# mengcaopku/DCNet

Hardware: AMD Instinct MI355X
Metric: clips/sec (T=8, 416x416, bs8) fwd+bwd (higher is better)
Workload: dtype f32; 1 GPU; T=8 416x416 bs8/GPU L=20 fp32, 64 img/GPU/step as pairs, fwd+5 losses+bwd+RMSprop; arith=f16x2-split MFMA, fp32 accumulate, parallelism=dp1, ranks_seen=1, reducer=none, step=hipGraph replay (fwd+losses+bwd+RMSprop), sampler=mt

## Files before the change

dcnet_amd/csrc/coattn.hip:

```cpp
#include "igemm.h"
#include "prof.h"
#include "coattn.h"

int tn_gemm_batched(const float* A, int lda, long long a_bs, const float* B, int ldb, long long b_bs,
                    float* C, int ldc, long long c_bs, const float* row_scale,
                    int M, int m_ld, int N, int K, int batch, int accumulate, hipStream_t stream,
                    const unsigned* amax_a = nullptr, const unsigned* amax_b = nullptr);

namespace {

constexpr int EXP_ROWS = 32;

typedef _Float16 f16x4c_t __attribute__((ext_vector_type(4)));
constexpr float E_SPLIT_SCALE = 8192.f;
template <bool SPLIT>
__global__ __launch_bounds__(256) void exp_sums_kernel(float* __restrict__ E, int hw, int ldE, float t,
                                                       float* __restrict__ rsum, float* __restrict__ colpart) {
  __shared__ float red[4][EXP_ROWS];
  const int b = blockIdx.y, rb = blockIdx.x;
  const int i0 = rb * EXP_ROWS;
  float* e = E + ((size_t)b * hw + i0) * ldE;
  float racc[EXP_ROWS];
#pragma unroll
  for (int r = 0; r < EXP_ROWS; ++r) racc[r] = 0.f;
// ... 16 lines not shown
          const f16x4c_t l = {(_Float16)(ts[0] - (float)h[0]), (_Float16)(ts[1] - (float)h[1]), (_Float16)(ts[2] - (float)h[2]),
                              (_Float16)(ts[3] - (float)h[3])};
          unsigned char* run = reinterpret_cast<unsigned char*>(e + (size_t)r * ldE + (j & ~7)) + (j & 4) * 2;
          *reinterpret_cast<f16x4c_t*>(run) = h;
          *reinterpret_cast<f16x4c_t*>(run + 16) = l;
        } else {
          *reinterpret_cast<f32x4*>(e + (size_t)r * ldE + j) = o;
        }
        cs += o; racc[r] += (o[0] + o[1]) + (o[2] + o[3]);
      }
    }
    *reinterpret_cast<f32x4*>(colpart + ((size_t)rb * gridDim.y + b) * ldE + j) = cs;
  }
  const int lane = threadIdx.x & 63, wave = threadIdx.x >> 6;
#pragma unroll
  for (int r = 0; r < EXP_ROWS; ++r) {
    const float s = wave_sum(racc[r]);
    if (lane == 0) red[wave][r] = s;
  }
  __syncthreads();
  if (threadIdx.x < EXP_ROWS && i0 + threadIdx.x < hw)
    rsum[(size_t)b * hw + i0 + threadIdx.x] = 1.f / (red[0][threadIdx.x] + red[1][threadIdx.x] + red[2][threadIdx.x] + red[3][threadIdx.x]);
}

__global__ __launch_bounds__(256) void colsum_inv_kernel(const float* __restrict__ colpart, int nrb, int b, int hw, int ldE,
                                                         float* __restrict__ cinv) {
  const int j = blockIdx.x * 256 + threadIdx.x, bb = blockIdx.y;
  if (j >= hw) return;
  float s = 0.f;
  for (int rb = 0; rb < nrb; ++rb) s += colpart[((size_t)rb * b + bb) * ldE + j];
  cinv[(size_t)bb * hw + j] = 1.f / s;
}

enum { AM_ONE = 0, AM_DO1, AM_DO2, AM_DO1S, AM_DO2S, AM_DA, AM_DP1, AM_DP2, AM_SLOTS };
__global__ __launch_bounds__(256) void amax_init_kernel(unsigned* __restrict__ w) {
  for (int i = threadIdx.x; i < AM_SLOTS * DCN_AMAX_WORDS; i += 256) w[i] = i < DCN_AMAX_WORDS ? 0x3F800000u : 0u;
}

__global__ __launch_bounds__(256) void rowdot_scale_kernel(const float* __restrict__ d, int ldd, int64_t bsd,
                                                           const float* __restrict__ o, int ldo, int64_t bso, int hw,
                                                           const float* __restrict__ inv, int64_t rows, int c,
                                                           float* __restrict__ delta, float* __restrict__ ds,
                                                           unsigned* __restrict__ amax_d, unsigned* __restrict__ amax_ds) {
  __shared__ float red[4];
  const int lane = threadIdx.x & 63;
  const int64_t row = (int64_t)blockIdx.x * 4 + (threadIdx.x >> 6);
  float vmax = 0.f, s = 0.f;
  if (row < rows) {
    const int64_t bb = row / hw, i = row - bb * hw;
    s = inv[row];
    float acc = 0.f;
    for (int k = lane * 4; k < c; k += 256) {
      const f32x4 dv = *reinterpret_cast<const f32x4*>(d + bb * bsd + i * ldd + k);
      const f32x4 ov = *reinterpret_cast<const f32x4*>(o + bb * bso + i * ldo + k);
      acc += dv[0] * ov[0] + dv[1] * ov[1] + dv[2] * ov[2] + dv[3] * ov[3];
      *reinterpret_cast<f32x4*>(ds + row * c + k) = dv * s;
      vmax = fmaxf(fmaxf(vmax, fmaxf(fabsf(dv[0]), fabsf(dv[1]))), fmaxf(fabsf(dv[2]), fabsf(dv[3])));
    }
    acc = wave_sum(acc);
    if (lane == 0) delta[row] = acc;
  }
  const float vs = wave_max(vmax * s);
  amax_update_block(amax_d, vmax, red);
  __syncthreads();
  amax_update_block(amax_ds, vs, red);
}

template <bool ESPLIT, bool OSPLIT = false>
__global__ __launch_bounds__(256) void dA_kernel(const float* __restrict__ E, float* __restrict__ dP1, const float* __restrict__ dP2,
                                                 const float* __restrict__ rinv, const float* __restrict__ cinv,
                                                 const float* __restrict__ d1, const float* __restrict__ d2,
                                                 int hw, int ldE, float t, int64_t total4, unsigned* __restrict__ amax_da) {
  __shared__ float red[4];
  float vmax = 0.f;
  const int l4 = ldE >> 2;
  float s_out = 1.f;
  if constexpr (OSPLIT) {
    const int be = (int)((amax_read(amax_da) >> 23) & 0xFF);
    int ex = (be == 0 || be == 255) ? 0 : 14 - (be - 126);
    ex = ex > 100 ? 100 : (ex < -100 ? -100 : ex);
    s_out = __uint_as_float((unsigned)(ex + 127) << 23);
  }
  for (int64_t idx = (int64_t)blockIdx.x * 256 + threadIdx.x; idx < total4; idx += (int64_t)gridDim.x * 256) {
    const int64_t row = idx / l4;
    const int j = (int)(idx - row * l4) * 4;
    const int64_t bb = row / hw;
    f32x4 e;
    if constexpr (ESPLIT) {
      const unsigned char* run = reinterpret_cast<const unsigned char*>(E + row * ldE + (j & ~7)) + (j & 4) * 2;
      const f16x4c_t h = *reinterpret_cast<const f16x4c_t*>(run), l = *reinterpret_cast<const f16x4c_t*>(run + 16);
#pragma unroll
      for (int k = 0; k < 4; ++k) e[k] = ((float)h[k] + (float)l[k]) * (1.f / E_SPLIT_SCALE);
    } else {
      e = *reinterpret_cast<const f32x4*>(E + row * ldE + j);
    }
    const f32x4 p1 = *reinterpret_cast<const f32x4*>(dP1 + row * ldE + j);
    const f32x4 p2 = *reinterpret_cast<const f32x4*>(dP2 + row * ldE + j);
    const float ri = rinv[row], di = d1[row];
    f32x4 o;
#pragma unroll
    for (int k = 0; k < 4; ++k) {
      float v = 0.f;
      if (j + k < hw) v = t * e[k] * ((p1[k] - di) * ri + (p2[k] - d2[bb * hw + j + k]) * cinv[bb * hw + j + k]);
      o[k] = v;
    }
    if constexpr (OSPLIT) {
      const f32x4 ts = o * s_out;
      const f16x4c_t h = {(_Float16)ts[0], (_Float16)ts[1], (_Float16)ts[2], (_Float16)ts[3]};
      const f16x4c_t l = {(_Float16)(ts[0] - (float)h[0]), (_Float16)(ts[1] - (float)h[1]), (_Float16)(ts[2] - (float)h[2]),
                          (_Float16)(ts[3] - (float)h[3])};
      unsigned char* run = reinterpret_cast<unsigned char*>(dP1 + row * ldE + (j & ~7)) + (j & 4) * 2;
      *reinterpret_cast<f16x4c_t*>(run) = h;
      *reinterpret_cast<f16x4c_t*>(run + 16) = l;
    } else {
      *reinterpret_cast<f32x4*>(dP1 + row * ldE + j) = o;
      vmax = fmaxf(fmaxf(vmax, fmaxf(fabsf(o[0]), fabsf(o[1]))), fmaxf(fabsf(o[2]), fabsf(o[3])));
    }
  }
  if constexpr (!OSPLIT) amax_update_block(amax_da, vmax, red);
}

__global__ __launch_bounds__(64) void da_bound_kernel(const unsigned* __restrict__ a1, const unsigned* __restrict__ a2, float t,
                                                      unsigned* __restrict__ out) {
  const float b = 2.f * t * (__uint_as_float(amax_read(a1)) + __uint_as_float(amax_read(a2)));
  out[threadIdx.x & (DCN_AMAX_WORDS - 1)] = __float_as_uint(b);
}

inline int ld_pad(int hw) { return (hw + 31) / 32 * 32; }

void gemm_params(IgemmParams& p, const float* A, int lda, long long a_bs, const float* B, int ldb, long long b_bs,
                 float* C, int ldc, long long c_bs, int M, int N, int K, int batch) {
  p = IgemmParams{};
  p.osy = p.osx = p.isy = p.isx = 1; p.dense_out = 1;
  p.in = A; p.ldi = lda; p.in_bs = a_bs; p.wt = B; p.ldw = ldb; p.wt_bs = b_bs; p.out = C; p.ldo = ldc; p.out_bs = c_bs;
  p.ldr = ldc;
  p.N = 1; p.Hi = 1; p.Wi = M; p.Ho = 1; p.Wo = M; p.Hs = 1; p.Ws = M; p.M = M;
// ... 29 lines not shown
  return (int64_t)cdiv(hw, EXP_ROWS) * b * ld_pad(hw) + AM_SLOTS * DCN_AMAX_WORDS;
}
extern "C" int64_t dcn_coattn_e_size(int b, int hw) { return (int64_t)b * hw * ld_pad(hw); }
extern "C" int64_t dcn_coattn_saved_size(int b, int hw, int c) {
  return dcn_coattn_e_size(b, hw) + (on_gemm3(b, hw, c) ? (int64_t)2 * b * hw * c : 0);
}

extern "C" int dcn_coattn_fwd(const float* f1, const float* f2, int ldf, int64_t bsf, float* f1_attn, float* f2_attn, int ldo,
                              int64_t bso, float* E, float* rinv, float* cinv, float* ws,
                              int b, int hw, int c, float temperature, void* stream_) {
  hipStream_t stream = (hipStream_t)stream_;
  DCN_CHECK_ARG(f1 && f2 && f1_attn && E && rinv && cinv && ws, "coattn_fwd: null pointer");
  DCN_CHECK_ARG(b > 0 && hw > 0 && c > 0 && c % 32 == 0, "coattn_fwd: bad shape (c=%d must be a multiple of 32)", c);
  if (ldf <= 0) ldf = c;
  if (ldo <= 0) ldo = c;
  DCN_CHECK_ARG(ldf % 4 == 0 && ldo % 4 == 0, "coattn_fwd: ldf/ldo must be multiples of 4");
  if (bsf <= 0) bsf = (int64_t)hw * ldf;
  if (bso <= 0) bso = (int64_t)hw * ldo;
  DCN_CHECK_ARG(bsf % 4 == 0 && bso % 4 == 0, "coattn_fwd: batch strides must be multiples of 4");
  const int ldE = ld_pad(hw);
  unsigned* am = reinterpret_cast<unsigned*>(ws + (int64_t)cdiv(hw, EXP_ROWS) * b * ldE);
  hipLaunchKernelGGL(amax_init_kernel, dim3(1), dim3(256), 0, stream, am);
  DCN_CHECK_LAUNCH("coattn amax_init");
  const unsigned* one = am + AM_ONE * DCN_AMAX_WORDS;
  const int nrb = cdiv(hw, EXP_ROWS);
  const long long bsE = (long long)hw * ldE;
  if (on_gemm3(b, hw, c)) {
    float* f1s = E + dcn_coattn_e_size(b, hw);
    float* f2s = f1s + (int64_t)b * hw * c;
    const long long bss = (long long)hw * c;
    int rc = gemm3_presplit(f1, ldf, bsf, f1s, c, bss, b, hw, c, one, stream);
    if (rc) return rc;
    if ((rc = gemm3_presplit(f2, ldf, bsf, f2s, c, bss, b, hw, c, one, stream))) return rc;
    if ((rc = gemm3_launch(f1s, c, bss, 0, f2s, c, bss, 0, E, ldE, bsE, nullptr, 0, hw, hw, c, b, 0, one, one, stream))) return rc;
    const int pid = prof_begin(12, (double)b * hw * ldE * 8.0, stream);
    hipLaunchKernelGGL(exp_sums_kernel<true>, dim3(nrb, b), dim3(256), 0, stream, E, hw, ldE, temperature, rinv, ws);
    prof_end(pid, stream);
    DCN_CHECK_LAUNCH("exp_sums");
    hipLaunchKernelGGL(colsum_inv_kernel, dim3(cdiv(hw, 256), b), dim3(256), 0, stream, ws, nrb, b, hw, ldE, cinv);
    DCN_CHECK_LAUNCH("colsum_inv");
    if ((rc = gemm3_launch(E, ldE, bsE, 0, f2s, c, bss, 1, f1_attn, ldo, bso, rinv, hw, hw, c, hw, b, 0, one, one, stream))) return rc;
    if (f2_attn) rc = gemm3_launch(E, ldE, bsE, 1, f1s, c, bss, 1, f2_attn, ldo, bso, cinv, hw, hw, c, hw, b, 0, one, one, stream);
    return rc;
  }
  IgemmParams p;
  gemm_params(p, f1, ldf, bsf, f2, ldf, bsf, E, ldE, (long long)hw * ldE, hw, hw, c, b);
  p.amax_a = one; p.amax_b = one;
  int rc = igemm_launch(p, stream);
  if (rc) return rc;
  const int pid = prof_begin(12, (double)b * hw * ldE * 8.0, stream);
  hipLaunchKernelGGL(exp_sums_kernel<false>, dim3(nrb, b), dim3(256), 0, stream, E, hw, ldE, temperature, rinv, ws);
  prof_end(pid, stream);
  DCN_CHECK_LAUNCH("exp_sums");
  hipLaunchKernelGGL(colsum_inv_kernel, dim3(cdiv(hw, 256), b), dim3(256), 0, stream, ws, nrb, b, hw, ldE, cinv);
  DCN_CHECK_LAUNCH("colsum_inv");
  gemm_params(p, E, ldE, (long long)hw * ldE, f2, ldf, bsf, f1_attn, ldo, bso, hw, c, ldE, b);
  p.bmode = 1; p.kvalid = hw; p.row_scale = rinv; p.amax_a = one; p.amax_b = one;
  rc = igemm_launch(p, stream);
  if (rc) return rc;
  if (f2_attn)
    rc = tn_gemm_batched(E, ldE, (long long)hw * ldE, f1, ldf, bsf, f2_attn, ldo, bso,
                         cinv, hw, ldE, c, hw, b, 0, stream, one, one);
  return rc;
}

extern "C" int64_t dcn_coattn_bwd_ws(int b, int hw, int c) {
  return (int64_t)2 * b * hw * ld_pad(hw) + (int64_t)2 * b * hw * c + (int64_t)2 * b * hw + AM_SLOTS * DCN_AMAX_WORDS +
         (on_gemm3(b, hw, c) ? (int64_t)2 * b * hw * c + 4 : 0);
}

extern "C" int dcn_coattn_bwd(const float* f1, const float* f2, int ldf, int64_t bsf,
                              const float* d_f1_attn, const float* d_f2_attn, int lddo, int64_t bsdo,
                              const float* f1_attn, const float* f2_attn, int ldo, int64_t bso,
                              const float* E, const float* rinv, const float* cinv,
                              float* d_f1, float* d_f2, int lddf, int64_t bsdf, int accumulate, float* ws,
                              int b, int hw, int c, float temperature, void* stream_) {
  hipStream_t stream = (hipStream_t)stream_;
  DCN_CHECK_ARG(f1 && f2 && d_f1_attn && d_f2_attn && f1_attn && f2_attn && E && rinv && cinv && d_f1 && d_f2 && ws,
                "coattn_bwd: null pointer");
  DCN_CHECK_ARG(b > 0 && hw > 0 && c > 0 && c % 32 == 0, "coattn_bwd: bad shape");
  if (ldf <= 0) ldf = c;
  if (ldo <= 0) ldo = c;
  if (lddo <= 0) lddo = c;
  if (lddf <= 0) lddf = c;
  if (bsf <= 0) bsf = (int64_t)hw * ldf;
  if (bso <= 0) bso = (int64_t)hw * ldo;
  if (bsdo <= 0) bsdo = (int64_t)hw * lddo;
  if (bsdf <= 0) bsdf = (int64_t)hw * lddf;
  const int ldE = ld_pad(hw);
  const long long rows = (long long)b * hw;
  float* dP1 = ws;
  float* dP2 = dP1 + rows * ldE;
  float* dO1s = dP2 + rows * ldE;
  float* dO2s = dO1s + rows * c;
  float* del1 = dO2s + rows * c;
  float* del2 = del1 + rows;
  unsigned* am = reinterpret_cast<unsigned*>(del2 + rows);
  hipLaunchKernelGGL(amax_init_kernel, dim3(1), dim3(256), 0, stream, am);
  DCN_CHECK_LAUNCH("coattn amax_init");
  auto slot = [&](int i) { return am + i * DCN_AMAX_WORDS; };
  hipLaunchKernelGGL(rowdot_scale_kernel, dim3(cdiv(rows, 4)), dim3(256), 0, stream, d_f1_attn, lddo, bsdo, f1_attn, ldo, bso, hw, rinv, rows, c, del1, dO1s,
                     slot(AM_DO1), slot(AM_DO1S));
  DCN_CHECK_LAUNCH("rowdot_scale");
  hipLaunchKernelGGL(rowdot_scale_kernel, dim3(cdiv(rows, 4)), dim3(256), 0, stream, d_f2_attn, lddo, bsdo, f2_attn, ldo, bso, hw, cinv, rows, c, del2, dO2s,
                     slot(AM_DO2), slot(AM_DO2S));
  DCN_CHECK_LAUNCH("rowdot_scale");
  const int64_t total4 = rows * (ldE / 4);
  int64_t g = (total4 + 255) / 256; if (g > 8192) g = 8192;
  if (g > 1024) g = 1024;
  const long long bsE = (long long)hw * ldE;
  if (on_gemm3(b, hw, c)) {
    float* dO1p = reinterpret_cast<float*>(((uintptr_t)(am + AM_SLOTS * DCN_AMAX_WORDS) + 15) & ~(uintptr_t)15);
    float* dO2p = dO1p + rows * c;
    const float* f1s = E + dcn_coattn_e_size(b, hw);
    const float* f2s = f1s + rows * c;
    const long long bss = (long long)hw * c;
    int rc;
    if ((rc = gemm3_presplit(d_f1_attn, lddo, bsdo, dO1p, c, bss, b, hw, c, slot(AM_DO1), stream))) return rc;
    if ((rc = gemm3_presplit(d_f2_attn, lddo, bsdo, dO2p, c, bss, b, hw, c, slot(AM_DO2), stream))) return rc;
    if ((rc = gemm3_presplit(dO1s, c, bss, dO1s, c, bss, b, hw, c, slot(AM_DO1S), stream))) return rc;
    if ((rc = gemm3_presplit(dO2s, c, bss, dO2s, c, bss, b, hw, c, slot(AM_DO2S), stream))) return rc;
    if ((rc = gemm3_launch(dO1p, c, bss, 0, f2s, c, bss, 0, dP1, ldE, bsE, nullptr, 0, hw, hw, c, b, 0, slot(AM_DO1), slot(AM_ONE), stream, slot(AM_DP1)))) return rc;
    if ((rc = gemm3_launch(f1s, c, bss, 0, dO2p, c, bss, 0, dP2, ldE, bsE, nullptr, 0, hw, hw, c, b, 0, slot(AM_ONE), slot(AM_DO2), stream, slot(AM_DP2)))) return rc;
    hipLaunchKernelGGL(da_bound_kernel, dim3(1), dim3(64), 0, stream, slot(AM_DP1), slot(AM_DP2), temperature, slot(AM_DA));
    DCN_CHECK_LAUNCH("dA bound");
    const int pid_da = prof_begin(31, (double)total4 * 16.0 * 4.0, stream);
    hipLaunchKernelGGL((dA_kernel<true, true>), dim3((int)g), dim3(256), 0, stream, E, dP1, dP2, rinv, cinv, del1, del2, hw, ldE, temperature, total4, slot(AM_DA));
    prof_end(pid_da, stream);
    DCN_CHECK_LAUNCH("dA");
    if ((rc = gemm3_launch(dP1, ldE, bsE, 0, f2s, c, bss, 1, d_f1, lddf, bsdf, nullptr, 0, hw, c, hw, b, accumulate, slot(AM_DA), slot(AM_ONE), stream))) return rc;
    if ((rc = gemm3_launch(E, ldE, bsE, 0, dO2s, c, bss, 1, d_f1, lddf, bsdf, nullptr, 0, hw, c, hw, b, 1, slot(AM_ONE), slot(AM_DO2S), stream))) return rc;
    if ((rc = gemm3_launch(dP1, ldE, bsE, 1, f1s, c, bss, 1, d_f2, lddf, bsdf, nullptr, 0, hw, c, hw, b, accumulate, slot(AM_DA), slot(AM_ONE), stream))) return rc;
    return gemm3_launch(E, ldE, bsE, 1, dO1s, c, bss, 1, d_f2, lddf, bsdf, nullptr, 0, hw, c, hw, b, 1, slot(AM_ONE), slot(AM_DO1S), stream);
  }
  IgemmParams p;
  int rc;
  gemm_params(p, d_f1_attn, lddo, bsdo, f2, ldf, bsf, dP1, ldE, (long long)hw * ldE, hw, hw, c, b);
  p.amax_a = slot(AM_DO1); p.amax_b = slot(AM_ONE);
  if ((rc = igemm_launch(p, stream))) return rc;
  gemm_params(p, f1, ldf, bsf, d_f2_attn, lddo, bsdo, dP2, ldE, (long long)hw * ldE, hw, hw, c, b);
  p.amax_a = slot(AM_ONE); p.amax_b = slot(AM_DO2);
  if ((rc = igemm_launch(p, stream))) return rc;
  const int pid_da = prof_begin(31, (double)total4 * 16.0 * 4.0, stream);
  hipLaunchKernelGGL(dA_kernel<false>, dim3((int)g), dim3(256), 0, stream, E, dP1, dP2, rinv, cinv, del1, del2, hw, ldE, temperature, total4, slot(AM_DA));
  prof_end(pid_da, stream);
  DCN_CHECK_LAUNCH("dA");
  gemm_params(p, dP1, ldE, (long long)hw * ldE, f2, ldf, bsf, d_f1, lddf, bsdf, hw, c, ldE, b);
  p.bmode = 1; p.kvalid = hw; p.accumulate = accumulate; p.amax_a = slot(AM_DA); p.amax_b = slot(AM_ONE);
  if ((rc = igemm_launch(p, stream))) return rc;
  gemm_params(p, E, ldE, (long long)hw * ldE, dO2s, c, (long long)hw * c, d_f1, lddf, bsdf, hw, c, ldE, b);
  p.bmode = 1; p.kvalid = hw; p.accumulate = 1; p.amax_a = slot(AM_ONE); p.amax_b = slot(AM_DO2S);
  if ((rc = igemm_launch(p, stream))) return rc;
  rc = tn_gemm_batched(dP1, ldE, (long long)hw * ldE, f1, ldf, bsf, d_f2, lddf, bsdf,
                       nullptr, hw, ldE, c, hw, b, accumulate, stream, slot(AM_DA), slot(AM_ONE));
  if (rc) return rc;
  return tn_gemm_batched(E, ldE, (long long)hw * ldE, dO1s, c, (long long)hw * c, d_f2, lddf, bsdf,
                         nullptr, hw, ldE, c, hw, b, 1, stream, slot(AM_ONE), slot(AM_DO1S));
}
```

dcnet_amd/csrc/gemm3.hip:

```cpp
#include "igemm.h"
#include "prof.h"

namespace {

typedef _Float16 f16x8_t __attribute__((ext_vector_type(8)));
typedef short s16x4 __attribute__((ext_vector_type(4)));
typedef short s16x8 __attribute__((ext_vector_type(8)));
typedef __attribute__((address_space(3))) void lds_void;

#ifndef G3_ABL
#define G3_ABL 0
#endif
constexpr unsigned G3_OOB = 0x80000000u;
constexpr int G3_BM = 256, G3_BN = 256, G3_STAGES = 4;
constexpr int G3_TILE = 256 * 64;
constexpr int G3_STAGE = 2 * G3_TILE;
constexpr int G3_LDS = G3_STAGES * G3_STAGE;

__device__ __forceinline__ float g3_pow2_scale(unsigned amax_bits) {
  const int be = (int)((amax_bits >> 23) & 0xFF);
  if (be == 0 || be == 255) return 1.f;
  int e = 14 - (be - 126);
  e = e > 100 ? 100 : (e < -100 ? -100 : e);
  return __uint_as_float((unsigned)(e + 127) << 23);
}

struct G3Params {
  const float* A; const float* B; float* C;
  long long a_bs, b_bs, c_bs;
  int lda, ldb, ldc;
  int M, N, K;
  int a_rows, b_rows;
  int a_cols, b_cols;
  int tiles_m, tiles_n;
  const float* row_scale; long long rs_bs;
  int accumulate;
  const unsigned* amax_a; const unsigned* amax_b;
  unsigned* amax_out;
  int var;
  int abl;
};

__device__ __forceinline__ int g3_tswz(int krow) { return (krow & 1) | ((krow & 2) << 1); }

template <bool AT, bool BT, bool H1 = false>
__global__ __launch_bounds__(512, 1) void gemm3_kernel(const G3Params p) {
  extern __shared__ __attribute__((aligned(1024))) unsigned char smem3g[];
  const int tid = threadIdx.x, lane = tid & 63;
  const int wave = __builtin_amdgcn_readfirstlane(tid >> 6);
  const int wm = wave >> 2, wn = wave & 3;
  const int per_batch = p.tiles_m * p.tiles_n;
  const int lin = xcd_remap(blockIdx.x, gridDim.x);
  const int batch = __builtin_amdgcn_readfirstlane(lin / per_batch), t_ = lin - batch * per_batch;
  const int bm = __builtin_amdgcn_readfirstlane(t_ / p.tiles_n), bn = t_ - bm * p.tiles_n;
  const int m0 = bm * G3_BM, n0 = bn * G3_BN;
  const int kslices = (p.K + 15) >> 4;

  const float* a_base = p.A + batch * p.a_bs + (AT ? 0 : (long long)m0 * p.lda);
  const float* b_base = p.B + batch * p.b_bs + (BT ? 0 : (long long)n0 * p.ldb);
  const int a_rows_left = AT ? p.a_rows : p.a_rows - m0, b_rows_left = BT ? p.b_rows : p.b_rows - n0;
  const long long a_bytes = ((long long)(a_rows_left - 1) * p.lda + p.a_cols) * 4, b_bytes = ((long long)(b_rows_left - 1) * p.ldb + p.b_cols) * 4;
  const __amdgpu_buffer_rsrc_t a_rs = __builtin_amdgcn_make_buffer_rsrc((void*)a_base, 0, a_bytes > 0x7FFFFFF0LL ? 0x7FFFFFF0 : (int)a_bytes, 0x00020000);
  const __amdgpu_buffer_rsrc_t b_rs = __builtin_amdgcn_make_buffer_rsrc((void*)b_base, 0, b_bytes > 0x7FFFFFF0LL ? 0x7FFFFFF0 : (int)b_bytes, 0x00020000);

  unsigned voff[4];
  int sstep_a, sstep_b;
#pragma unroll
  for (int e = 0; e < 2; ++e) {
    const int j = 2 * wave + e;
    if (AT) {
      voff[e] = (unsigned)((long long)j * p.lda * 4 + m0 * 4 + ((lane ^ g3_tswz(j)) << 4));
      if (m0 + ((lane ^ g3_tswz(j)) << 2) >= p.a_cols) voff[e] = G3_OOB;
    } else {
      const int row = 16 * j + (lane >> 2), c = (lane & 3) ^ ((row >> 2) & 3);
// ... 122 lines not shown
    asm volatile("" ::: "memory");
    if (G3_ABL && (p.abl & 4)) {
#pragma unroll
      for (int mi = 0; mi < 4; ++mi) { asm volatile("" :: "v"(ah[mi]), "v"(al[mi])); }
#pragma unroll
      for (int ni = 0; ni < 2; ++ni) { asm volatile("" :: "v"(bh[ni]), "v"(bl[ni])); }
    } else {
      __builtin_amdgcn_s_setprio(1);
      if constexpr (!H1) {
#pragma unroll
        for (int mi = 0; mi < 4; ++mi)
#pragma unroll
          for (int ni = 0; ni < 2; ++ni) acc[mi][ni] = __builtin_amdgcn_mfma_f32_32x32x16_f16(al[mi], bh[ni], acc[mi][ni], 0, 0, 0);
        if (p.var == 2) issue_b();
#pragma unroll
        for (int mi = 0; mi < 4; ++mi)
#pragma unroll
          for (int ni = 0; ni < 2; ++ni) acc[mi][ni] = __builtin_amdgcn_mfma_f32_32x32x16_f16(ah[mi], bl[ni], acc[mi][ni], 0, 0, 0);
      } else if (p.var == 2) issue_b();
#pragma unroll
      for (int mi = 0; mi < 4; ++mi)
#pragma unroll
        for (int ni = 0; ni < 2; ++ni) acc[mi][ni] = __builtin_amdgcn_mfma_f32_32x32x16_f16(ah[mi], bh[ni], acc[mi][ni], 0, 0, 0);
      __builtin_amdgcn_s_setprio(0);
    }
    if (p.var == 1) issue_b();
    if (wm == 0) asm volatile("s_waitcnt vmcnt(%0)" :: "n"((G3_STAGES - 2) * 4) : "memory");
  }
  if (wm == 0) __builtin_amdgcn_s_barrier();
  asm volatile("s_waitcnt vmcnt(0)" ::: "memory");

  const float dq = 1.f / (g3_pow2_scale(amax_read(p.amax_a)) * g3_pow2_scale(amax_read(p.amax_b)));
  float* __restrict__ cb = p.C + batch * p.c_bs;
  const float* rs = p.row_scale ? p.row_scale + batch * p.rs_bs : nullptr;
  float vmax = 0.f;
#pragma unroll
  for (int mi = 0; mi < 4; ++mi)
#pragma unroll
    for (int r = 0; r < 16; ++r) {
      const int m = m0 + wm * 128 + mi * 32 + 4 * g + (r & 3) + 8 * (r >> 2);
      if (m >= p.M) continue;
      const float f = rs ? dq * rs[m] : dq;
#pragma unroll
      for (int ni = 0; ni < 2; ++ni) {
        const int n = n0 + wn * 64 + ni * 32 + (lane & 31);
        if (n >= p.N) continue;
        float v = acc[mi][ni][r] * f;
        float* dst = cb + (long long)m * p.ldc + n;
        if (p.accumulate) v += *dst;
        *dst = v;
        vmax = fmaxf(vmax, fabsf(v));
      }
    }
  if (p.amax_out) {
    vmax = wave_max(vmax);
    if (lane == 0) amax_update(p.amax_out, vmax, blockIdx.x * 8 + wave);
  }
}

__global__ __launch_bounds__(256) void presplit_kernel(const float* __restrict__ src, int ld, long long bs, float* __restrict__ dst, int ldd,
                                                        long long bsd, int rows, int c, long long total8, const unsigned* __restrict__ amax) {
  const float s = g3_pow2_scale(amax_read(amax));
  const int c8 = c >> 3;
  for (long long i = (long long)blockIdx.x * 256 + threadIdx.x; i < total8; i += (long long)gridDim.x * 256) {
    const long long row_all = i / c8; const int o = (int)(i - row_all * c8);
    const long long b = row_all / rows; const int row = (int)(row_all - b * rows);
    const float* sp = src + b * bs + (long long)row * ld + o * 8;
    const f32x4 x0 = *reinterpret_cast<const f32x4*>(sp) * s, x1 = *reinterpret_cast<const f32x4*>(sp + 4) * s;
    f16x8_t h, l;
#pragma unroll
    for (int e = 0; e < 4; ++e) { h[e] = (_Float16)x0[e]; h[4 + e] = (_Float16)x1[e]; }
#pragma unroll
    for (int e = 0; e < 4; ++e) { l[e] = (_Float16)(x0[e] - (float)h[e]); l[4 + e] = (_Float16)(x1[e] - (float)h[4 + e]); }
    float* dp = dst + b * bsd + (long long)row * ldd + o * 8;
    *reinterpret_cast<f16x8_t*>(dp) = h;
    *reinterpret_cast<f16x8_t*>(dp + 4) = l;
  }
}

DCN_KNOB(g_gemm3, "Gemm3", 1, "gemm3.hip: the co-attention products on pre-split operands (0 = implicit-GEMM / weight-gradient tiles; + 256 * v = schedule variant v; + 16 * bits = timing ablations, results WRONG)",
         nullptr, "-DG3_ABL=1", G3_ABL != 0, [](int v) { return (v & 0xF0) != 0; });
DCN_KNOB(g_gemm3_h1, "H1gemm3", 1, "gemm3.hip: one f16 piece per operand in the bf16 precision modes (0 = both pieces, fp32-accurate co-attention)");

template <bool AT, bool BT, bool H1>
int launch3g_(const G3Params& p, int grid, hipStream_t stream) {
  static DcnPerDeviceFlag attr_once;
  if (attr_once.first()) {
    (void)hipFuncSetAttribute(reinterpret_cast<const void*>(&gemm3_kernel<AT, BT, H1>), hipFuncAttributeMaxDynamicSharedMemorySize, G3_LDS);
  }
  hipLaunchKernelGGL((gemm3_kernel<AT, BT, H1>), dim3(grid), dim3(512), G3_LDS, stream, p);
  return DCN_OK;
}
template <bool AT, bool BT>
int launch3g(const G3Params& p, int grid, hipStream_t stream) {
  if (g_gemm3_h1 && igemm_precision() == 2) return launch3g_<AT, BT, true>(p, grid, stream);
  return launch3g_<AT, BT, false>(p, grid, stream);
}

}

int gemm3_variant() { const int v = g_gemm3 >> 8; return (v == 1 || v == 2) ? v : 0; }
extern "C" int dcn_gemm3_variant() { return gemm3_variant(); }

bool gemm3_applicable(int M, int N, int K, int batch) {
  return g_gemm3 && (igemm_precision() == 4 || igemm_precision() == 2) && M >= 512 && N >= 256 && K >= 64 && batch >= 1;
}

int gemm3_presplit(const float* src, int ld, long long bs, float* dst, int ldd, long long bsd, int batch, int rows, int c,
                   const unsigned* amax, hipStream_t stream) {
  DCN_CHECK_ARG(src && dst && amax && c % 8 == 0 && ld % 4 == 0 && ldd % 4 == 0 && bs % 4 == 0 && bsd % 4 == 0, "gemm3_presplit: bad argument");
  const long long total8 = (long long)batch * rows * (c / 8);
  long long g = (total8 + 255) / 256; if (g > 16384) g = 16384;
  hipLaunchKernelGGL(presplit_kernel, dim3((int)g), dim3(256), 0, stream, src, ld, bs, dst, ldd, bsd, rows, c, total8, amax);
  DCN_CHECK_LAUNCH("gemm3_presplit");
  return DCN_OK;
}

int gemm3_launch(const float* A, int lda, long long a_bs, int at, const float* B, int ldb, long long b_bs, int bt,
                 float* C, int ldc, long long c_bs, const float* row_scale, long long rs_bs,
                 int M, int N, int K, int batch, int accumulate, const unsigned* amax_a, const unsigned* amax_b, hipStream_t stream,
                 unsigned* amax_out) {
  DCN_CHECK_ARG(A && B && C && amax_a && amax_b, "gemm3: null pointer");
  DCN_CHECK_ARG(lda % 4 == 0 && ldb % 4 == 0 && a_bs % 4 == 0 && b_bs % 4 == 0 && (((uintptr_t)A | (uintptr_t)B) & 15) == 0, "gemm3: 16-byte rows");
  G3Params p{};
  p.A = A; p.B = B; p.C = C; p.a_bs = a_bs; p.b_bs = b_bs; p.c_bs = c_bs; p.lda = lda; p.ldb = ldb; p.ldc = ldc;
  p.M = M; p.N = N; p.K = K;
  const int k16 = (K + 15) / 16 * 16;
  p.a_rows = at ? K : M; p.b_rows = bt ? K : N;
  p.a_cols = at ? (M + 7) / 8 * 8 : k16; p.b_cols = bt ? (N + 7) / 8 * 8 : k16;
  DCN_CHECK_ARG(p.a_cols <= lda && p.b_cols <= ldb, "gemm3: rows shorter than the tile reads (lda=%d ldb=%d)", lda, ldb);
  p.tiles_m = cdiv(M, G3_BM); p.tiles_n = cdiv(N, G3_BN);
  p.row_scale = row_scale; p.rs_bs = rs_bs; p.accumulate = accumulate; p.amax_a = amax_a; p.amax_b = amax_b; p.amax_out = amax_out; p.abl = (g_gemm3 >> 4) & 15; p.var = gemm3_variant();
  const int grid = p.tiles_m * p.tiles_n * batch;
  const int pid = prof_begin(40, 2.0 * batch * (double)M * N * K, stream);
  int rc;
  if (at) rc = bt ? launch3g<true, true>(p, grid, stream) : DCN_ERR_ARG;
  else rc = bt ? launch3g<false, true>(p, grid, stream) : launch3g<false, false>(p, grid, stream);
  prof_end(pid, stream);
  DCN_CHECK_ARG(rc == DCN_OK, "gemm3: no A^T . B^T form");
  DCN_CHECK_LAUNCH("gemm3");
  return DCN_OK;
}

extern "C" int dcn_gemm3_supported(int m, int n, int k, int batch) { return gemm3_applicable(m, n, k, batch) ? 1 : 0; }

extern "C" int dcn_gemm3_presplit(const float* src, int ld, int64_t bs, float* dst, int ldd, int64_t bsd, int batch, int rows, int c,
                                  const uint32_t* amax, void* stream) {
  return gemm3_presplit(src, ld, bs, dst, ldd, bsd, batch, rows, c, amax, (hipStream_t)stream);
}

extern "C" int dcn_gemm3(const float* a, int lda, int64_t a_bs, int a_t, const float* b, int ldb, int64_t b_bs, int b_t,
                         float* c, int ldc, int64_t c_bs, const float* row_scale, int64_t rs_bs,
                         int m, int n, int k, int batch, int accumulate, const uint32_t* amax_a, const uint32_t* amax_b, void* stream) {
  DCN_CHECK_ARG(m > 0 && n > 0 && k > 0 && batch > 0, "gemm3: empty problem");
  return gemm3_launch(a, lda, a_bs, a_t, b, ldb, b_bs, b_t, c, ldc, c_bs, row_scale, rs_bs, m, n, k, batch, accumulate, amax_a, amax_b,
                      (hipStream_t)stream, nullptr);
}
```

dcnet_amd/csrc/igemm.h:

```cpp
#pragma once
#include "common.h"

#define IGEMM_MAX_TAPS 16


struct IgemmParams {
  const float* in;
  const float* wt;
  const float* f8;
  const unsigned* amax_a;
  const unsigned* amax_b;
  const void* wt16;
  const float* b_scale;
  unsigned* amax_out;
  float* out;
  const float* scale;
  const float* shift;
  const float* residual;
  float* stats;
  const float* row_scale;
  int batch;
  long long in_bs, wt_bs, out_bs;
  int bmode;
  int kvalid;
// ... 27 lines not shown
int conv3_launch(const IgemmParams& p, int gran, hipStream_t stream);
bool conv3x_takes(const IgemmParams& p, int gran);
int conv3x_launch(const IgemmParams& p, int gran, hipStream_t stream);
int conv3b_bm(int M, int Co, int Wi);
bool conv3b_takes(const IgemmParams& p);
int conv3b_launch(const IgemmParams& p, int out_f32, hipStream_t stream);

bool conv1_applicable(const IgemmParams& p, int precision, int gran);
int conv1_launch(const IgemmParams& p, int gran, hipStream_t stream);
int conv1_tile_of(long long rows, int Co, int ntaps, int Ci, int stats, int gran, int storage16);
int conv1b_grid_m(int M, int Co, int ntaps, int s1_w = 0);
int conv1b_launch(const IgemmParams& p, int out_f32, hipStream_t stream);
int conv1q_grid_m(int M, int Co);
int conv1q_launch(const IgemmParams& p, int out_f32, hipStream_t stream);
bool conv2b_takes(int M, int Co, int ntaps);
int conv2b_launch(const IgemmParams& p, int out_f32, hipStream_t stream);


bool stem_applicable(const IgemmParams& p, const float* scratch);
int stem_launch(const IgemmParams& p, float* scratch, hipStream_t stream);

bool dgrad2_applicable(int n, int h, int wd, int cin, int cout, int ksize, int stride, int accumulate);
struct DcnBnTap { const float* y; const float* mean; const float* invstd; const float* gamma; const float* beta; int act; float slope;
                  float* stats; int stats_rows; };
int nconv1_launch_b16(int mode, const void* x, int ldi, const void* w16, void* y, int ldo, float* stats, int stats_rows,
                      int n, int h, int wd, int stride, hipStream_t stream);
int dgrad2_launch_b16(const void* dy, int lddy, const void* wt16, void* dx, int n, int h, int wd, int cin, int accumulate, hipStream_t stream);
int dgrad2_grid(int n, int h, int wd, int cin);
int dgrad2_launch(const float* dy, int lddy, const float* wt, float* dx, int n, int h, int wd, int cin, int accumulate,
                  const uint32_t* amax_dy, const uint32_t* amax_w, const DcnBnTap* tap, hipStream_t stream);
bool gemm3_applicable(int M, int N, int K, int batch);
int gemm3_presplit(const float* src, int ld, long long bs, float* dst, int ldd, long long bsd, int batch, int rows, int c,
                   const unsigned* amax, hipStream_t stream);
int gemm3_launch(const float* A, int lda, long long a_bs, int at, const float* B, int ldb, long long b_bs, int bt,
                 float* C, int ldc, long long c_bs, const float* row_scale, long long rs_bs,
                 int M, int N, int K, int batch, int accumulate, const unsigned* amax_a, const unsigned* amax_b, hipStream_t stream,
                 unsigned* amax_out = nullptr);
int igemm_precision();
extern int g_abl;
extern int g_wsplit;
struct DcnPreAct { const float* scale; const float* shift; int act; float slope; };
bool nconv1_applicable(int mode, int n, int h, int wd, int cin, int cout, int ksize, int stride);
int nconv1_launch(int mode, const float* x, int ldi, const float* w, float* y, int ldo, float* stats, int stats_rows,
                  int n, int h, int wd, int stride, const uint32_t* amax_x, const uint32_t* amax_w, const DcnPreAct* pre, hipStream_t stream);
```

Before: 87.13 clips/s.

## Fuse softmax exp and row/column sums into co-attention GEMM epilogue

The affinity GEMM epilogue now applies exp(t*a - t), writes E directly in the split f16 pair format, and produces per-tile row and column partial sums. A small kernel turns these into the inverse row and column sums, replacing the separate exp_sums and colsum passes over E. In backward, the dP GEMMs use the pre-scaled gradients, so two presplit passes go away and dA uses a prescaled formula. rowdot_scale also handles four rows per wave to cut the block count. The trade-offs are more register and LDS pressure in the GEMM epilogue and slightly different rounding.

Result: no change. 87.61 clips/s (median of 6 runs) (+0.6%).

```diff
diff --git a/dcnet_amd/csrc/coattn.hip b/dcnet_amd/csrc/coattn.hip
--- a/dcnet_amd/csrc/coattn.hip
+++ b/dcnet_amd/csrc/coattn.hip
@@ -72,11 +72,24 @@
   cinv[(size_t)bb * hw + j] = 1.f / s;
 }
 
+__global__ __launch_bounds__(256) void tile_sums_inv_kernel(const float* __restrict__ rowpart, int tiles_n, const float* __restrict__ colpart,
+                                                            int tiles_m, int b, int hw, int ldE, float* __restrict__ rinv, float* __restrict__ cinv) {
+  const int j = blockIdx.x * 256 + threadIdx.x, bb = blockIdx.y;
+  if (j >= hw) return;
+  const bool col = blockIdx.z != 0;
+  const float* part = col ? colpart : rowpart;
+  const int n = col ? tiles_m : tiles_n, ld = col ? ldE : hw;
+  float s = 0.f;
+  for (int k = 0; k < n; ++k) s += part[((size_t)k * b + bb) * ld + j];
+  (col ? cinv : rinv)[(size_t)bb * hw + j] = 1.f / s;
+}
+
 enum { AM_ONE = 0, AM_DO1, AM_DO2, AM_DO1S, AM_DO2S, AM_DA, AM_DP1, AM_DP2, AM_SLOTS };
 __global__ __launch_bounds__(256) void amax_init_kernel(unsigned* __restrict__ w) {
   for (int i = threadIdx.x; i < AM_SLOTS * DCN_AMAX_WORDS; i += 256) w[i] = i < DCN_AMAX_WORDS ? 0x3F800000u : 0u;
 }
 
+constexpr int ROWDOT_RPW = 4;
 __global__ __launch_bounds__(256) void rowdot_scale_kernel(const float* __restrict__ d, int ldd, int64_t bsd,
                                                            const float* __restrict__ o, int ldo, int64_t bso, int hw,
                                                            const float* __restrict__ inv, int64_t rows, int c,
@@ -84,29 +97,41 @@
                                                            unsigned* __restrict__ amax_d, unsigned* __restrict__ amax_ds) {
   __shared__ float red[4];
   const int lane = threadIdx.x & 63;
-  const int64_t row = (int64_t)blockIdx.x * 4 + (threadIdx.x >> 6);
-  float vmax = 0.f, s = 0.f;
-  if (row < rows) {
+  const int64_t row0 = ((int64_t)blockIdx.x * 4 + (threadIdx.x >> 6)) * ROWDOT_RPW;
+  float vmax = 0.f, vs = 0.f;
+  float acc[ROWDOT_RPW], s[ROWDOT_RPW];
+  const float* dp[ROWDOT_RPW]; const float* op[ROWDOT_RPW];
+#pragma unroll
+  for (int r = 0; r < ROWDOT_RPW; ++r) {
+    const int64_t row = row0 + r < rows ? row0 + r : rows - 1;
     const int64_t bb = row / hw, i = row - bb * hw;
-    s = inv[row];
-    float acc = 0.f;
-    for (int k = lane * 4; k < c; k += 256) {
-      const f32x4 dv = *reinterpret_cast<const f32x4*>(d + bb * bsd + i * ldd + k);
-      const f32x4 ov = *reinterpret_cast<const f32x4*>(o + bb * bso + i * ldo + k);
-      acc += dv[0] * ov[0] + dv[1] * ov[1] + dv[2] * ov[2] + dv[3] * ov[3];
-      *reinterpret_cast<f32x4*>(ds + row * c + k) = dv * s;
-      vmax = fmaxf(fmaxf(vmax, fmaxf(fabsf(dv[0]), fabsf(dv[1]))), fmaxf(fabsf(dv[2]), fabsf(dv[3])));
-    }
-    acc = wave_sum(acc);
-    if (lane == 0) delta[row] = acc;
-  }
-  const float vs = wave_max(vmax * s);
+    dp[r] = d + bb * bsd + i * ldd; op[r] = o + bb * bso + i * ldo;
+    s[r] = inv[row]; acc[r] = 0.f;
+  }
+  for (int k = lane * 4; k < c; k += 256) {
+    f32x4 dv[ROWDOT_RPW], ov[ROWDOT_RPW];
+#pragma unroll
+    for (int r = 0; r < ROWDOT_RPW; ++r) { dv[r] = *reinterpret_cast<const f32x4*>(dp[r] + k); ov[r] = *reinterpret_cast<const f32x4*>(op[r] + k); }
+#pragma unroll
+    for (int r = 0; r < ROWDOT_RPW; ++r) {
+      if (row0 + r >= rows) continue;
+      acc[r] += dv[r][0] * ov[r][0] + dv[r][1] * ov[r][1] + dv[r][2] * ov[r][2] + dv[r][3] * ov[r][3];
+      *reinterpret_cast<f32x4*>(ds + (row0 + r) * c + k) = dv[r] * s[r];
+      const float m = fmaxf(fmaxf(fabsf(dv[r][0]), fabsf(dv[r][1])), fmaxf(fabsf(dv[r][2]), fabsf(dv[r][3])));
+      vmax = fmaxf(vmax, m); vs = fmaxf(vs, m * s[r]);
+    }
+  }
+#pragma unroll
+  for (int r = 0; r < ROWDOT_RPW; ++r) {
+    const float a = wave_sum(acc[r]);
+    if (lane == 0 && row0 + r < rows) delta[row0 + r] = a;
+  }
   amax_update_block(amax_d, vmax, red);
   __syncthreads();
   amax_update_block(amax_ds, vs, red);
 }
 
-template <bool ESPLIT, bool OSPLIT = false>
+template <bool ESPLIT, bool OSPLIT = false, bool PRESCALED = false>
 __global__ __launch_bounds__(256) void dA_kernel(const float* __restrict__ E, float* __restrict__ dP1, const float* __restrict__ dP2,
                                                  const float* __restrict__ rinv, const float* __restrict__ cinv,
                                                  const float* __restrict__ d1, const float* __restrict__ d2,
@@ -141,7 +166,10 @@
 #pragma unroll
     for (int k = 0; k < 4; ++k) {
       float v = 0.f;
-      if (j + k < hw) v = t * e[k] * ((p1[k] - di) * ri + (p2[k] - d2[bb * hw + j + k]) * cinv[bb * hw + j + k]);
+      if (j + k < hw) {
+        const float dj = d2[bb * hw + j + k], cj = cinv[bb * hw + j + k];
+        v = PRESCALED ? t * e[k] * ((p1[k] - di * ri) + (p2[k] - dj * cj)) : t * e[k] * ((p1[k] - di) * ri + (p2[k] - dj) * cj);
+      }
       o[k] = v;
     }
     if constexpr (OSPLIT) {
@@ -237,13 +265,22 @@
     int rc = gemm3_presplit(f1, ldf, bsf, f1s, c, bss, b, hw, c, one, stream);
     if (rc) return rc;
     if ((rc = gemm3_presplit(f2, ldf, bsf, f2s, c, bss, b, hw, c, one, stream))) return rc;
-    if ((rc = gemm3_launch(f1s, c, bss, 0, f2s, c, bss, 0, E, ldE, bsE, nullptr, 0, hw, hw, c, b, 0, one, one, stream))) return rc;
-    const int pid = prof_begin(12, (double)b * hw * ldE * 8.0, stream);
-    hipLaunchKernelGGL(exp_sums_kernel<true>, dim3(nrb, b), dim3(256), 0, stream, E, hw, ldE, temperature, rinv, ws);
-    prof_end(pid, stream);
-    DCN_CHECK_LAUNCH("exp_sums");
-    hipLaunchKernelGGL(colsum_inv_kernel, dim3(cdiv(hw, 256), b), dim3(256), 0, stream, ws, nrb, b, hw, ldE, cinv);
-    DCN_CHECK_LAUNCH("colsum_inv");
+    if (gemm3_epilogues()) {
+      const int tm = cdiv(hw, 256);
+      G3Epi ep{};
+      ep.mode = 1; ep.t = temperature; ep.cols = ldE; ep.colpart = ws; ep.rowpart = ws + (int64_t)tm * b * ldE;
+      if ((rc = gemm3_launch(f1s, c, bss, 0, f2s, c, bss, 0, E, ldE, bsE, nullptr, 0, hw, hw, c, b, 0, one, one, stream, nullptr, &ep))) return rc;
+      hipLaunchKernelGGL(tile_sums_inv_kernel, dim3(cdiv(hw, 256), b, 2), dim3(256), 0, stream, ep.rowpart, tm, ep.colpart, tm, b, hw, ldE, rinv, cinv);
+      DCN_CHECK_LAUNCH("tile_sums_inv");
+    } else {
+      if ((rc = gemm3_launch(f1s, c, bss, 0, f2s, c, bss, 0, E, ldE, bsE, nullptr, 0, hw, hw, c, b, 0, one, one, stream))) return rc;
+      const int pid = prof_begin(12, (double)b * hw * ldE * 8.0, stream);
+      hipLaunchKernelGGL(exp_sums_kernel<true>, dim3(nrb, b), dim3(256), 0, stream, E, hw, ldE, temperature, rinv, ws);
+      prof_end(pid, stream);
+      DCN_CHECK_LAUNCH("exp_sums");
+      hipLaunchKernelGGL(colsum_inv_kernel, dim3(cdiv(hw, 256), b), dim3(256), 0, stream, ws, nrb, b, hw, ldE, cinv);
+      DCN_CHECK_LAUNCH("colsum_inv");
+    }
     if ((rc = gemm3_launch(E, ldE, bsE, 0, f2s, c, bss, 1, f1_attn, ldo, bso, rinv, hw, hw, c, hw, b, 0, one, one, stream))) return rc;
     if (f2_attn) rc = gemm3_launch(E, ldE, bsE, 1, f1s, c, bss, 1, f2_attn, ldo, bso, cinv, hw, hw, c, hw, b, 0, one, one, stream);
     return rc;
@@ -270,6 +307,8 @@
 }
 
 extern "C" int64_t dcn_coattn_bwd_ws(int b, int hw, int c) {
+  if (on_gemm3(b, hw, c) && gemm3_epilogues())
+    return (int64_t)2 * b * hw * ld_pad(hw) + (int64_t)2 * b * hw * c + (int64_t)2 * b * hw + AM_SLOTS * DCN_AMAX_WORDS;
   return (int64_t)2 * b * hw * ld_pad(hw) + (int64_t)2 * b * hw * c + (int64_t)2 * b * hw + AM_SLOTS * DCN_AMAX_WORDS +
          (on_gemm3(b, hw, c) ? (int64_t)2 * b * hw * c + 4 : 0);
 }
@@ -304,10 +343,10 @@
   hipLaunchKernelGGL(amax_init_kernel, dim3(1), dim3(256), 0, stream, am);
   DCN_CHECK_LAUNCH("coattn amax_init");
   auto slot = [&](int i) { return am + i * DCN_AMAX_WORDS; };
-  hipLaunchKernelGGL(rowdot_scale_kernel, dim3(cdiv(rows, 4)), dim3(256), 0, stream, d_f1_attn, lddo, bsdo, f1_attn, ldo, bso, hw, rinv, rows, c, del1, dO1s,
+  hipLaunchKernelGGL(rowdot_scale_kernel, dim3(cdiv(rows, 4 * ROWDOT_RPW)), dim3(256), 0, stream, d_f1_attn, lddo, bsdo, f1_attn, ldo, bso, hw, rinv, rows, c, del1, dO1s,
                      slot(AM_DO1), slot(AM_DO1S));
   DCN_CHECK_LAUNCH("rowdot_scale");
-  hipLaunchKernelGGL(rowdot_scale_kernel, dim3(cdiv(rows, 4)), dim3(256), 0, stream, d_f2_attn, lddo, bsdo, f2_attn, ldo, bso, hw, cinv, rows, c, del2, dO2s,
+  hipLaunchKernelGGL(rowdot_scale_kernel, dim3(cdiv(rows, 4 * ROWDOT_RPW)), dim3(256), 0, stream, d_f2_attn, lddo, bsdo, f2_attn, ldo, bso, hw, cinv, rows, c, del2, dO2s,
                      slot(AM_DO2), slot(AM_DO2S));
   DCN_CHECK_LAUNCH("rowdot_scale");
   const int64_t total4 = rows * (ldE / 4);
@@ -321,18 +360,31 @@
     const float* f2s = f1s + rows * c;
     const long long bss = (long long)hw * c;
     int rc;
-    if ((rc = gemm3_presplit(d_f1_attn, lddo, bsdo, dO1p, c, bss, b, hw, c, slot(AM_DO1), stream))) return rc;
-    if ((rc = gemm3_presplit(d_f2_attn, lddo, bsdo, dO2p, c, bss, b, hw, c, slot(AM_DO2), stream))) return rc;
-    if ((rc = gemm3_presplit(dO1s, c, bss, dO1s, c, bss, b, hw, c, slot(AM_DO1S), stream))) return rc;
-    if ((rc = gemm3_presplit(dO2s, c, bss, dO2s, c, bss, b, hw, c, slot(AM_DO2S), stream))) return rc;
-    if ((rc = gemm3_launch(dO1p, c, bss, 0, f2s, c, bss, 0, dP1, ldE, bsE, nullptr, 0, hw, hw, c, b, 0, slot(AM_DO1), slot(AM_ONE), stream, slot(AM_DP1)))) return rc;
-    if ((rc = gemm3_launch(f1s, c, bss, 0, dO2p, c, bss, 0, dP2, ldE, bsE, nullptr, 0, hw, hw, c, b, 0, slot(AM_ONE), slot(AM_DO2), stream, slot(AM_DP2)))) return rc;
-    hipLaunchKernelGGL(da_bound_kernel, dim3(1), dim3(64), 0, stream, slot(AM_DP1), slot(AM_DP2), temperature, slot(AM_DA));
-    DCN_CHECK_LAUNCH("dA bound");
-    const int pid_da = prof_begin(31, (double)total4 * 16.0 * 4.0, stream);
-    hipLaunchKernelGGL((dA_kernel<true, true>), dim3((int)g), dim3(256), 0, stream, E, dP1, dP2, rinv, cinv, del1, del2, hw, ldE, temperature, total4, slot(AM_DA));
-    prof_end(pid_da, stream);
-    DCN_CHECK_LAUNCH("dA");
+    if (gemm3_epilogues()) {
+      if ((rc = gemm3_presplit(dO1s, c, bss, dO1s, c, bss, b, hw, c, slot(AM_DO1S), stream))) return rc;
+      if ((rc = gemm3_presplit(dO2s, c, bss, dO2s, c, bss, b, hw, c, slot(AM_DO2S), stream))) return rc;
+      if ((rc = gemm3_launch(dO1s, c, bss, 0, f2s, c, bss, 0, dP1, ldE, bsE, nullptr, 0, hw, hw, c, b, 0, slot(AM_DO1S), slot(AM_ONE), stream, slot(AM_DP1)))) return rc;
+      if ((rc = gemm3_launch(f1s, c, bss, 0, dO2s, c, bss, 0, dP2, ldE, bsE, nullptr, 0, hw, hw, c, b, 0, slot(AM_ONE), slot(AM_DO2S), stream, slot(AM_DP2)))) return rc;
+      hipLaunchKernelGGL(da_bound_kernel, dim3(1), dim3(64), 0, stream, slot(AM_DP1), slot(AM_DP2), temperature, slot(AM_DA));
+      DCN_CHECK_LAUNCH("dA bound");
+      const int pid_da = prof_begin(31, (double)total4 * 16.0 * 4.0, stream);
+      hipLaunchKernelGGL((dA_kernel<true, true, true>), dim3((int)g), dim3(256), 0, stream, E, dP1, dP2, rinv, cinv, del1, del2, hw, ldE, temperature, total4, slot(AM_DA));
+      prof_end(pid_da, stream);
+      DCN_CHECK_LAUNCH("dA");
+    } else {
+      if ((rc = gemm3_presplit(d_f1_attn, lddo, bsdo, dO1p, c, bss, b, hw, c, slot(AM_DO1), stream))) return rc;
+      if ((rc = gemm3_presplit(d_f2_attn, lddo, bsdo, dO2p, c, bss, b, hw, c, slot(AM_DO2), stream))) return rc;
+      if ((rc = gemm3_presplit(dO1s, c, bss, dO1s, c, bss, b, hw, c, slot(AM_DO1S), stream))) return rc;
+      if ((rc = gemm3_presplit(dO2s, c, bss, dO2s, c, bss, b, hw, c, slot(AM_DO2S), stream))) return rc;
+      if ((rc = gemm3_launch(dO1p, c, bss, 0, f2s, c, bss, 0, dP1, ldE, bsE, nullptr, 0, hw, hw, c, b, 0, slot(AM_DO1), slot(AM_ONE), stream, slot(AM_DP1)))) return rc;
+      if ((rc = gemm3_launch(f1s, c, bss, 0, dO2p, c, bss, 0, dP2, ldE, bsE, nullptr, 0, hw, hw, c, b, 0, slot(AM_ONE), slot(AM_DO2), stream, slot(AM_DP2)))) return rc;
+      hipLaunchKernelGGL(da_bound_kernel, dim3(1), dim3(64), 0, stream, slot(AM_DP1), slot(AM_DP2), temperature, slot(AM_DA));
+      DCN_CHECK_LAUNCH("dA bound");
+      const int pid_da = prof_begin(31, (double)total4 * 16.0 * 4.0, stream);
+      hipLaunchKernelGGL((dA_kernel<true, true>), dim3((int)g), dim3(256), 0, stream, E, dP1, dP2, rinv, cinv, del1, del2, hw, ldE, temperature, total4, slot(AM_DA));
+      prof_end(pid_da, stream);
+      DCN_CHECK_LAUNCH("dA");
+    }
     if ((rc = gemm3_launch(dP1, ldE, bsE, 0, f2s, c, bss, 1, d_f1, lddf, bsdf, nullptr, 0, hw, c, hw, b, accumulate, slot(AM_DA), slot(AM_ONE), stream))) return rc;
     if ((rc = gemm3_launch(E, ldE, bsE, 0, dO2s, c, bss, 1, d_f1, lddf, bsdf, nullptr, 0, hw, c, hw, b, 1, slot(AM_ONE), slot(AM_DO2S), stream))) return rc;
     if ((rc = gemm3_launch(dP1, ldE, bsE, 1, f1s, c, bss, 1, d_f2, lddf, bsdf, nullptr, 0, hw, c, hw, b, accumulate, slot(AM_DA), slot(AM_ONE), stream))) return rc;
diff --git a/dcnet_amd/csrc/gemm3.hip b/dcnet_amd/csrc/gemm3.hip
--- a/dcnet_amd/csrc/gemm3.hip
+++ b/dcnet_amd/csrc/gemm3.hip
@@ -39,7 +39,19 @@
   unsigned* amax_out;
   int var;
   int abl;
+  G3Epi epi; int nbatch;
 };
+
+constexpr int DPP_XOR1 = 0xB1, DPP_XOR2 = 0x4E, DPP_HALF_MIRROR = 0x141, DPP_MIRROR = 0x140;
+template <int CTRL>
+__device__ __forceinline__ unsigned g3_dpp(unsigned v) { return (unsigned)__builtin_amdgcn_mov_dpp((int)v, CTRL, 0xF, 0xF, true); }
+template <int CTRL>
+__device__ __forceinline__ float g3_dpp_add(float v) { return v + __uint_as_float(g3_dpp<CTRL>(__float_as_uint(v))); }
+
+__device__ __forceinline__ unsigned g3_split_pack(float sv) {
+  const _Float16 h = (_Float16)sv, l = (_Float16)(sv - (float)h);
+  return (unsigned)__builtin_bit_cast(unsigned short, h) | ((unsigned)__builtin_bit_cast(unsigned short, l) << 16);
+}
 
 __device__ __forceinline__ int g3_tswz(int krow) { return (krow & 1) | ((krow & 2) << 1); }
 
@@ -228,6 +240,56 @@
 
   const float dq = 1.f / (g3_pow2_scale(amax_read(p.amax_a)) * g3_pow2_scale(amax_read(p.amax_b)));
   float* __restrict__ cb = p.C + batch * p.c_bs;
+  if constexpr (!AT && !BT && !H1) {
+    if (p.epi.mode) {
+      const G3Epi& q = p.epi;
+      const int ln = lane & 31;
+      const bool odd = ln & 1;
+      const int piece = (ln >> 3) * 32 + (odd ? 16 : 0) + (ln & 6) * 2;
+      const unsigned lane_off = (unsigned)(4 * g * p.ldc * 4 + piece);
+      float* red = reinterpret_cast<float*>(smem3g);
+      __syncthreads();
+      float csum[2] = {0.f, 0.f};
+#pragma unroll
+      for (int mi = 0; mi < 4; ++mi)
+#pragma unroll
+        for (int r = 0; r < 16; ++r) {
+          const int ml = wm * 128 + mi * 32 + 4 * g + (r & 3) + 8 * (r >> 2);
+          const bool mok = m0 + ml < p.M;
+          float rsum = 0.f;
+#pragma unroll
+          for (int ni = 0; ni < 2; ++ni) {
+            const int nb = n0 + wn * 64 + ni * 32;
+            const float a = acc[mi][ni][r] * dq;
+            const float ev = expf(q.t * a - q.t); const float e = (mok && nb + ln < p.N) ? ev : 0.f;
+            rsum += e; csum[ni] += e;
+            const unsigned x = g3_split_pack(e * 8192.f), y = g3_dpp<DPP_XOR1>(x);
+            const unsigned o = odd ? ((y >> 16) | (x & 0xFFFF0000u)) : ((x & 0xFFFFu) | (y << 16));
+            unsigned char* rowbase = reinterpret_cast<unsigned char*>(cb + (long long)(m0 + wm * 128 + mi * 32 + (r & 3) + 8 * (r >> 2)) * p.ldc + nb);
+            if (mok && nb < q.cols) *reinterpret_cast<unsigned*>(rowbase + lane_off) = o;
+          }
+          rsum = g3_dpp_add<DPP_MIRROR>(g3_dpp_add<DPP_HALF_MIRROR>(g3_dpp_add<DPP_XOR2>(g3_dpp_add<DPP_XOR1>(rsum))));
+          if ((lane & 15) == 0) red[(wn * 2 + ((lane >> 4) & 1)) * 256 + ml] = rsum;
+          __builtin_amdgcn_sched_barrier(0);
+        }
+#pragma unroll
+      for (int ni = 0; ni < 2; ++ni) {
+        csum[ni] += __shfl_xor(csum[ni], 32);
+        if (lane < 32) red[(8 + wm) * 256 + wn * 64 + ni * 32 + ln] = csum[ni];
+      }
+      __syncthreads();
+      if (tid < 256) {
+        float s = red[tid];
+#pragma unroll
+        for (int k = 1; k < 8; ++k) s += red[k * 256 + tid];
+        if (m0 + tid < p.M) q.rowpart[((long long)bn * p.nbatch + batch) * p.M + m0 + tid] = s;
+      } else {
+        const int c = tid - 256;
+        if (n0 + c < q.cols) q.colpart[((long long)bm * p.nbatch + batch) * q.cols + n0 + c] = red[8 * 256 + c] + red[9 * 256 + c];
+      }
+      return;
+    }
+  }
   const float* rs = p.row_scale ? p.row_scale + batch * p.rs_bs : nullptr;
   float vmax = 0.f;
 #pragma unroll
@@ -274,7 +336,7 @@
   }
 }
 
-DCN_KNOB(g_gemm3, "Gemm3", 1, "gemm3.hip: the co-attention products on pre-split operands (0 = implicit-GEMM / weight-gradient tiles; + 256 * v = schedule variant v; + 16 * bits = timing ablations, results WRONG)",
+DCN_KNOB(g_gemm3, "Gemm3", 1, "gemm3.hip: the co-attention products on pre-split operands (0 = implicit-GEMM / weight-gradient tiles; + 256 * v = schedule variant v; + 16 * bits = timing ablations, results WRONG; + 4096: the co-attention exponentiates in a pass of its own and multiplies by the unscaled gradients, as before the fused epilogue)",
          nullptr, "-DG3_ABL=1", G3_ABL != 0, [](int v) { return (v & 0xF0) != 0; });
 DCN_KNOB(g_gemm3_h1, "H1gemm3", 1, "gemm3.hip: one f16 piece per operand in the bf16 precision modes (0 = both pieces, fp32-accurate co-attention)");
 
@@ -289,13 +351,14 @@
 }
 template <bool AT, bool BT>
 int launch3g(const G3Params& p, int grid, hipStream_t stream) {
-  if (g_gemm3_h1 && igemm_precision() == 2) return launch3g_<AT, BT, true>(p, grid, stream);
+  if (g_gemm3_h1 && igemm_precision() == 2) return p.epi.mode ? DCN_ERR_ARG : launch3g_<AT, BT, true>(p, grid, stream);
   return launch3g_<AT, BT, false>(p, grid, stream);
 }
 
 }
 
-int gemm3_variant() { const int v = g_gemm3 >> 8; return (v == 1 || v == 2) ? v : 0; }
+int gemm3_variant() { const int v = (g_gemm3 >> 8) & 15; return (v == 1 || v == 2) ? v : 0; }
+bool gemm3_epilogues() { return !(g_gemm3 & 4096) && !(g_gemm3_h1 && igemm_precision() == 2); }
 extern "C" int dcn_gemm3_variant() { return gemm3_variant(); }
 
 bool gemm3_applicable(int M, int N, int K, int batch) {
@@ -315,8 +378,13 @@
 int gemm3_launch(const float* A, int lda, long long a_bs, int at, const float* B, int ldb, long long b_bs, int bt,
                  float* C, int ldc, long long c_bs, const float* row_scale, long long rs_bs,
                  int M, int N, int K, int batch, int accumulate, const unsigned* amax_a, const unsigned* amax_b, hipStream_t stream,
-                 unsigned* amax_out) {
+                 unsigned* amax_out, const G3Epi* epi) {
   DCN_CHECK_ARG(A && B && C && amax_a && amax_b, "gemm3: null pointer");
+  if (epi && epi->mode) {
+    DCN_CHECK_ARG(!at && !bt && !row_scale && !accumulate && !amax_out && epi->cols >= N && epi->cols <= ldc && epi->cols % 32 == 0 && ldc % 4 == 0,
+                  "gemm3: a split-form epilogue belongs to a plain NT product whose rows hold the padded columns");
+    DCN_CHECK_ARG(epi->mode == 1 && epi->rowpart && epi->colpart, "gemm3: epilogue mode %d, or no room for its sums", epi->mode);
+  }
   DCN_CHECK_ARG(lda % 4 == 0 && ldb % 4 == 0 && a_bs % 4 == 0 && b_bs % 4 == 0 && (((uintptr_t)A | (uintptr_t)B) & 15) == 0, "gemm3: 16-byte rows");
   G3Params p{};
   p.A = A; p.B = B; p.C = C; p.a_bs = a_bs; p.b_bs = b_bs; p.c_bs = c_bs; p.lda = lda; p.ldb = ldb; p.ldc = ldc;
@@ -327,6 +395,8 @@
   DCN_CHECK_ARG(p.a_cols <= lda && p.b_cols <= ldb, "gemm3: rows shorter than the tile reads (lda=%d ldb=%d)", lda, ldb);
   p.tiles_m = cdiv(M, G3_BM); p.tiles_n = cdiv(N, G3_BN);
   p.row_scale = row_scale; p.rs_bs = rs_bs; p.accumulate = accumulate; p.amax_a = amax_a; p.amax_b = amax_b; p.amax_out = amax_out; p.abl = (g_gemm3 >> 4) & 15; p.var = gemm3_variant();
+  if (epi) p.epi = *epi;
+  p.nbatch = batch;
   const int grid = p.tiles_m * p.tiles_n * batch;
   const int pid = prof_begin(40, 2.0 * batch * (double)M * N * K, stream);
   int rc;
diff --git a/dcnet_amd/csrc/igemm.h b/dcnet_amd/csrc/igemm.h
--- a/dcnet_amd/csrc/igemm.h
+++ b/dcnet_amd/csrc/igemm.h
@@ -83,10 +83,15 @@
 bool gemm3_applicable(int M, int N, int K, int batch);
 int gemm3_presplit(const float* src, int ld, long long bs, float* dst, int ldd, long long bsd, int batch, int rows, int c,
                    const unsigned* amax, hipStream_t stream);
+struct G3Epi {
+  int mode; float t; int cols;
+  float* rowpart; float* colpart;
+};
+bool gemm3_epilogues();
 int gemm3_launch(const float* A, int lda, long long a_bs, int at, const float* B, int ldb, long long b_bs, int bt,
                  float* C, int ldc, long long c_bs, const float* row_scale, long long rs_bs,
                  int M, int N, int K, int batch, int accumulate, const unsigned* amax_a, const unsigned* amax_b, hipStream_t stream,
-                 unsigned* amax_out = nullptr);
+                 unsigned* amax_out = nullptr, const G3Epi* epi = nullptr);
 int igemm_precision();
 extern int g_abl;
 extern int g_wsplit;
```
